# isarandi/metrabs

Measured on AMD Instinct MI355X. Metric: crops/sec (256px, 72 depth bins) at 1/2/4/8 MI355X; MPJPE vs ref, higher is better.
Workload: dtype f32

## Files before the change

include/metrabs_hip.h:

```cpp
#ifndef METRABS_HIP_H_
#define METRABS_HIP_H_

#include <stddef.h>
#include <stdint.h>

#ifdef __cplusplus
extern "C" {
#endif

#define MTR_VERSION 100

typedef void* mtr_stream_t;

enum mtr_dtype { MTR_F32 = 0, MTR_F16 = 1, MTR_BF16 = 2 };

enum mtr_layout {
  MTR_NCHW = 0,
  MTR_NHWC = 1
};

enum mtr_error {
  MTR_OK = 0,
  MTR_E_NULL = -1,
  MTR_E_SHAPE = -2,
// ... 172 lines not shown
                     const int32_t* row_start, const int32_t* sim_offsets, int n_images, int P, int A,
                     int J, const int32_t* edges, const float* mean_bones, int n_bones, int J_model,
                     const mtr_filter_params* params , void* workspace, size_t workspace_bytes,
                     int max_per_image, uint8_t* valid, int32_t* keep_idx, int32_t* keep_count,
                     mtr_stream_t stream);

int mtr_bias_act_nchw(void* y, int dtype, const float* bias , const void* residual, int act,
                      long long B, int C, int HW, mtr_stream_t stream);

int mtr_bias_act_rowmean_nchw(void* y, int dtype, const float* bias , int act, long long B,
                              int C, int HW, float* row_mean , mtr_stream_t stream);

int mtr_depthwise3x3_bias_act(const void* x, int dtype, const float* weight, const float* bias, int act,
                              long long B, int C, int H, int W, int stride, int pad, void* y,
                              float* row_mean, mtr_stream_t stream);
int mtr_depthwise3x3_bias_act_padded(const void* x, int dtype, const float* weight, const float* bias,
                                     int act, long long B, int C, int H, int W, int stride, int pad_top,
                                     int pad_left, int pad_bottom, int pad_right, void* y,
                                     float* row_mean, mtr_stream_t stream);

int mtr_depthwise5x5_bias_act_padded(const void* x, int dtype, const float* weight ,
                                     const float* bias, int act, long long B, int C, int H, int W,
                                     int stride, int pad_top, int pad_left, int pad_bottom, int pad_right,
                                     void* y, float* row_mean , mtr_stream_t stream);

int mtr_se_gate(const float* mean , const float* w1, const float* b1, const float* w2,
                const float* b2, int act, int gate_fn, int B, int C, int S, float* gate ,
                mtr_stream_t stream);

int mtr_conv1x1_bias_act(const void* x, int dtype, const float* weight, const float* bias,
                         const float* gate , const void* residual, int act, long long B,
                         int M, int K, int HW, void* y, mtr_stream_t stream);

int mtr_conv1x1_bias_act16(const void* x, int dtype, const void* weight, const float* bias,
                           const float* gate , const void* residual, int act, long long B,
                           int M, int K, int HW, void* y, mtr_stream_t stream);

int mtr_conv3x3_bias_act16(const void* x, int dtype, const void* weight , const float* bias,
                           const void* residual, int act, long long B, int Cin, int Cout, int H, int W, int stride,
                           void* y, mtr_stream_t stream);

size_t mtr_conv3x3_16_lds_bytes(long long B, int Cin, int Cout, int H, int W, int stride);

#ifdef __cplusplus
}
#endif
#endif
```

metrabs_amd/_lib.py:

```python
import ctypes
import os
from ctypes import POINTER, c_char_p, c_double, c_float, c_int, c_int32, c_size_t, c_uint8, c_void_p

LIB_PATH = os.path.join(os.path.dirname(os.path.abspath(__file__)), 'csrc', 'libmetrabs_hip.so')

MTR_F32, MTR_F16, MTR_BF16 = 0, 1, 2
MTR_NCHW, MTR_NHWC = 0, 1
MTR_WARP_PARAM_FLOATS = 36


class HeadParams(ctypes.Structure):
    _fields_ = [('proc_side', c_int32), ('stride_test', c_int32), ('centered_stride', c_int32),
                ('legacy_centered_stride_bug', c_int32), ('box_size_mm', c_float)]


class HeadOptions(ctypes.Structure):
    _fields_ = [('struct_size', ctypes.c_uint32),
                ('rt_tiles_per_workgroup', c_int32), ('groups_per_workgroup', c_int32),
                ('dma_staging', c_int32), ('rt_column_blocks', c_int32), ('rt_k_groups', c_int32),
                ('rt_loader', c_int32), ('rt_split_column_blocks', c_int32)]


def head_options(rt_tiles=0, groups_per_workgroup=0, dma_staging=-1, rt_column_blocks=0, rt_k_groups=0,
                 rt_loader=0, rt_split=0):
# ... 84 lines not shown
                                  c_void_p, c_void_p, c_void_p]),
    'mtr_postprocess_poses': (c_int, [c_void_p, c_void_p, c_void_p, c_void_p, c_void_p, c_int, c_void_p,
                                      c_int, c_void_p, c_void_p, c_void_p, c_int, c_int, c_int, c_int,
                                      c_void_p, c_void_p, c_void_p]),
    'mtr_linear_combine_points': (c_int, [c_void_p, c_void_p, c_int, c_int, c_int, c_void_p, c_void_p]),
    'mtr_warp_crops': (c_int, [c_void_p, c_void_p, c_void_p, c_int, c_int, c_int, c_void_p, c_int,
                               c_int, c_int, c_int, c_int, c_void_p, c_void_p]),
    'mtr_detector_geometry': (c_int, [c_int, c_int, c_int, POINTER(DetectorGeom)]),
    'mtr_detector_preprocess': (c_int, [c_void_p, c_int, c_int, c_int, POINTER(DetectorGeom), c_void_p,
                                        c_void_p]),
    'mtr_detector_preprocess_kernel': (c_int, [c_void_p, c_int, c_int, c_int, POINTER(DetectorGeom), c_int,
                                               c_void_p, c_void_p]),
    'mtr_detector_scale_boxes': (c_int, [c_void_p, c_int, POINTER(DetectorGeom), c_void_p, c_void_p]),
    'mtr_filter_poses_workspace_bytes': (ctypes.c_size_t, [c_int, c_int, c_int]),
    'mtr_filter_poses': (c_int, [c_void_p, c_void_p, c_void_p, c_void_p, c_void_p, c_int, c_int, c_int,
                                 c_int, c_void_p, c_void_p, c_int, c_int, POINTER(FilterParams), c_void_p,
                                 ctypes.c_size_t, c_int, c_void_p, c_void_p, c_void_p, c_void_p]),
    'mtr_depthwise3x3_bias_act': (c_int, [c_void_p, c_int, c_void_p, c_void_p, c_int, ctypes.c_longlong,
                                          c_int, c_int, c_int, c_int, c_int, c_void_p, c_void_p, c_void_p]),
    'mtr_depthwise3x3_bias_act_padded': (c_int, [c_void_p, c_int, c_void_p, c_void_p, c_int, ctypes.c_longlong,
                                                 c_int, c_int, c_int, c_int, c_int, c_int, c_int, c_int,
                                                 c_void_p, c_void_p, c_void_p]),
    'mtr_depthwise5x5_bias_act_padded': (c_int, [c_void_p, c_int, c_void_p, c_void_p, c_int, ctypes.c_longlong,
                                                 c_int, c_int, c_int, c_int, c_int, c_int, c_int, c_int,
                                                 c_void_p, c_void_p, c_void_p]),
    'mtr_bias_act_rowmean_nchw': (c_int, [c_void_p, c_int, c_void_p, c_int, ctypes.c_longlong, c_int, c_int,
                                          c_void_p, c_void_p]),
    'mtr_bias_act_nchw': (c_int, [c_void_p, c_int, c_void_p, c_void_p, c_int, ctypes.c_longlong, c_int,
                                  c_int, c_void_p]),
    'mtr_se_gate': (c_int, [c_void_p, c_void_p, c_void_p, c_void_p, c_void_p, c_int, c_int, c_int, c_int,
                            c_int, c_void_p, c_void_p]),
    'mtr_conv1x1_bias_act': (c_int, [c_void_p, c_int, c_void_p, c_void_p, c_void_p, c_void_p, c_int,
                                     ctypes.c_longlong, c_int, c_int, c_int, c_void_p, c_void_p]),
    'mtr_conv1x1_bias_act16': (c_int, [c_void_p, c_int, c_void_p, c_void_p, c_void_p, c_void_p, c_int,
                                       ctypes.c_longlong, c_int, c_int, c_int, c_void_p, c_void_p]),
    'mtr_conv3x3_bias_act16': (c_int, [c_void_p, c_int, c_void_p, c_void_p, c_void_p, c_int, ctypes.c_longlong,
                                       c_int, c_int, c_int, c_int, c_int, c_void_p, c_void_p]),
    'mtr_conv3x3_16_lds_bytes': (ctypes.c_size_t, [ctypes.c_longlong, c_int, c_int, c_int, c_int, c_int]),
}

_lib = None


def load(path=None):
    global _lib
    if _lib is not None and path is None:
        return _lib
    path = path or LIB_PATH
    import torch
    if not os.path.exists(path):
        raise RuntimeError(
            f'{path} not found: the HIP extension is not built. Run `python -m metrabs_amd.build` '
            f'(needs hipcc). metrabs_amd has no CPU fallback.')
    lib = ctypes.CDLL(path)
    for name, (restype, argtypes) in SIGNATURES.items():
        fn = getattr(lib, name)
        fn.restype = restype
        fn.argtypes = argtypes
    _lib = lib
    return lib


def check(code, what):
    if code != 0:
        msg = load().mtr_strerror(code).decode()
        raise RuntimeError(f'{what} failed: {msg} (code {code})')
# ... 22 lines not shown
```

metrabs_amd/backbones.py:

```python
import collections
import threading

import torch
import torch.nn.functional as F
from torch import nn


class DepthwiseConv2d(nn.Conv2d):

    use_miopen = False
    _backend_lock = threading.Lock()

    def forward(self, x):
        if x.is_cuda and not DepthwiseConv2d.use_miopen and torch.backends.cudnn.enabled:
            cudnn = torch.backends.cudnn
            with DepthwiseConv2d._backend_lock, cudnn.flags(
                    enabled=False, benchmark=cudnn.benchmark, deterministic=cudnn.deterministic,
                    allow_tf32=cudnn.allow_tf32):
                return super().forward(x)
        return super().forward(x)


class ConvBNAct(nn.Sequential):

# ... 49 lines not shown
            return False
        return (type(self.act) in (nn.SiLU, nn.ReLU) and type(self.gate) in self._GATE_NAMES
                and self.fc1.weight.dtype == torch.float32 and self.fc1.bias is not None
                and self.fc2.bias is not None and self.fc1.weight.is_cuda
                and self.fc1.in_channels % 4 == 0)


def _padded_conv(layers, name, cin, cout, k, stride, groups=1, act=nn.SiLU, bottomright=False):
    total = k - 1
    beg, end = total // 2, total - total // 2
    if bottomright:
        layers['padding'] = nn.ZeroPad2d((beg - 1, end + 1, beg - 1, end + 1))
        layers[name] = ConvBNAct(cin, cout, k, stride, groups=groups, act=act, padding=0)
    elif beg == end:
        layers[name] = ConvBNAct(cin, cout, k, stride, groups=groups, act=act, padding=beg)
    else:
        layers['padding'] = nn.ZeroPad2d((beg, end, beg, end))
        layers[name] = ConvBNAct(cin, cout, k, stride, groups=groups, act=act, padding=0)


class FusedMBConv(nn.Module):

    def __init__(self, cin, cout, expand, stride, bottomright=False):
        super().__init__()
        self.residual = stride == 1 and cin == cout
        mid = cin * expand
        layers = collections.OrderedDict()
        if expand == 1:
            _padded_conv(layers, '0', cin, cout, 3, stride, bottomright=bottomright)
        else:
            _padded_conv(layers, '0', cin, mid, 3, stride, bottomright=bottomright)
            layers['1'] = ConvBNAct(mid, cout, 1, 1, act=None)
        self.block = nn.Sequential(layers)

    def forward(self, x):
        return _block_plus_skip(self.block, x) if self.residual else self.block(x)


class MBConv(nn.Module):

    def __init__(self, cin, cout, expand, stride, k=3, bottomright=False):
        super().__init__()
        self.residual = stride == 1 and cin == cout
        mid = cin * expand
        layers = collections.OrderedDict()
        if mid != cin:
            layers['0'] = ConvBNAct(cin, mid, 1, 1)
        n = len(layers)
        _padded_conv(layers, str(n), mid, mid, k, stride, groups=mid, bottomright=bottomright)
        layers[str(n + 1)] = SqueezeExcite(mid, max(1, cin // 4))
        layers[str(n + 2)] = ConvBNAct(mid, cout, 1, 1, act=None)
        self.block = nn.Sequential(layers)

    def forward(self, x):
        return _block_plus_skip(self.block, x) if self.residual else self.block(x)


class Preproc(nn.Module):

    def forward(self, x):
        return x * 2 - 1


EFFNETV2 = {
    's': dict(stem=24, stages=[('f', 1, 1, 24, 24, 2), ('f', 4, 2, 24, 48, 4), ('f', 4, 2, 48, 64, 4),
                               ('m', 4, 2, 64, 128, 6), ('m', 6, 1, 128, 160, 9),
                               ('m', 6, 2, 160, 256, 15)], head=1280),
    'm': dict(stem=24, stages=[('f', 1, 1, 24, 24, 3), ('f', 4, 2, 24, 48, 5), ('f', 4, 2, 48, 80, 5),
                               ('m', 4, 2, 80, 160, 7), ('m', 6, 1, 160, 176, 14),
# ... 74 lines not shown
    layers += [ConvBNAct(cin, 960, 1, 1, act=nn.Hardswish), ConvBNAct(960, 1280, 1, 1, act=nn.Hardswish)]
    net = nn.Sequential(*layers)
    net.out_channels = 1280
    return net


def build_backbone(name):
    name = name.lower()
    if name in ('efficientnetv2-s', 'effnetv2-s', 'effv2s'):
        return efficientnetv2('s')
    if name in ('efficientnetv2-l', 'effnetv2-l', 'effv2l'):
        return efficientnetv2('l')
    if name in ('resnet18', 'resnet-18'):
        return resnet18()
    if name in ('mobilenetv3', 'mobilenetv3-large', 'mobilenet-v3'):
        return mobilenet_v3_large()
    raise ValueError(f'unknown backbone {name}')


_ACT_NAMES = {nn.SiLU: 'silu', nn.ReLU: 'relu', nn.Hardswish: 'hardswish'}


class ConvBiasAct(nn.Module):

    def __init__(self, conv, bias, act):
        super().__init__()
        self.conv = conv
        self.register_buffer('bias', bias.detach().float().contiguous())
        self.act = act
        self.act_name = None if act is None else _ACT_NAMES[type(act)]
        self.emit_mean = False
        self._mean = None
        self._gate = None
        self.last_path = None

    use_k13 = True
    k13_slower = frozenset({(960, 256, 64), (1536, 256, 64), (256, 1280, 64)})

    def k13_takes(self, x):
        c = self.conv
        if not (ConvBiasAct.use_k13 and not self.emit_mean and x.is_cuda and c.kernel_size == (1, 1)
                and c.stride == (1, 1) and c.padding == (0, 0) and c.dilation == (1, 1) and c.groups == 1
                and c.bias is None and c.padding_mode == 'zeros'):
            return False
        if torch.is_autocast_enabled('cuda') or (torch.is_grad_enabled() and c.weight.requires_grad):
            return False
        if x.dim() != 4 or (c.in_channels, c.out_channels, x.shape[2] * x.shape[3]) in ConvBiasAct.k13_slower:
            return False
        from . import kernels
        return kernels.conv1x1_supported(x, c.weight)

    use_k13h = True
    k13h_slower = frozenset({(192, 48, 4096), (256, 64, 1024), (1536, 256, 64), (256, 64, 9216), (768, 192, 576),
                             (1152, 224, 576), (1344, 224, 576), (1344, 384, 144), (2304, 384, 144),
                             (2304, 640, 144), (640, 3840, 144), (3840, 640, 144), (640, 1280, 144)})

    def k13h_takes(self, x):
        c = self.conv
        if not (ConvBiasAct.use_k13h and not self.emit_mean and x.is_cuda and x.dtype == c.weight.dtype
                and x.dtype in (torch.float16, torch.bfloat16) and c.kernel_size == (1, 1)
                and c.stride == (1, 1) and c.padding == (0, 0) and c.dilation == (1, 1) and c.groups == 1
                and c.bias is None and c.padding_mode == 'zeros'):
            return False
        if torch.is_autocast_enabled('cuda') or (torch.is_grad_enabled() and c.weight.requires_grad):
            return False
        if x.dim() != 4 or (c.in_channels, c.out_channels, x.shape[2] * x.shape[3]) in ConvBiasAct.k13h_slower:
            return False
        from . import kernels
        return kernels.conv1x1_16_supported(x, c.weight)

    def give_gate(self, x, gate):
        self._gate = (x, gate)

    def take_mean_f32(self, x):
        held, self._mean = self._mean, None
        if held is not None and held[0] is x:
            return held[1]
        return None

    def take_mean(self, x):
        m = self.take_mean_f32(x)
        return None if m is None else m.to(x.dtype).view(x.shape[0], x.shape[1], 1, 1)

    def forward(self, x, residual=None):
        held, self._gate = self._gate, None
        gate = held[1] if held is not None and held[0] is x else None
        w16 = self.conv.weight.dtype
        if x.dtype != w16 and w16 in (torch.float16, torch.bfloat16) and not torch.is_autocast_enabled(x.device.type):
            x = x.to(w16)
        if self.k13h_takes(x) and (residual is None or (residual.dtype == x.dtype and residual.is_contiguous()
                                                        and residual.data_ptr() % 16 == 0)):
            from . import kernels
            self.last_path = 'k13h' if gate is None else 'k13h_gate'
            return kernels.conv1x1_bias_act16(x, self.conv.weight, self.bias, self.act_name, gate=gate,
                                              residual=residual)
        if self.k13_takes(x) and (residual is None or (residual.dtype == x.dtype and residual.is_contiguous()
                                                       and residual.data_ptr() % 16 == 0)):
            from . import kernels
            self.last_path = 'k13' if gate is None else 'k13_gate'
            return kernels.conv1x1_bias_act(x, self.conv.weight, self.bias, self.act_name, gate=gate,
                                            residual=residual)
        self.last_path = 'library'
        if gate is not None:
            x = x * gate.to(x.dtype).view(x.shape[0], x.shape[1], 1, 1)
        return _library_conv_bias_act(self, x, residual)


def _library_conv_bias_act(mod, x, residual):
    y = mod.conv(x)
    hw_vec_ok = (y.shape[2] * y.shape[3]) % (16 // y.element_size()) == 0
    if y.is_cuda and y.is_contiguous() and hw_vec_ok and y.data_ptr() % 16 == 0 and (
            residual is None or (residual.dtype == y.dtype and residual.is_contiguous()
                                 and residual.data_ptr() % 16 == 0)):
        from . import kernels
        if getattr(mod, 'emit_mean', False) and residual is None:
            y, mean = kernels.bias_act_rowmean_(y, mod.bias, mod.act_name)
            mod._mean = (y, mean)
            return y
        return kernels.bias_act_(y, mod.bias, mod.act_name, residual)
    y = y + mod.bias.view(1, -1, 1, 1).to(y.dtype)
    y = y if mod.act is None else mod.act(y)
    return y if residual is None else residual + y


class Conv3x3BiasAct(nn.Module):

    use_k14h = True
    k14h_slower = frozenset({(64, 256, 2, 96, 96), (64, 64, 1, 64, 64)})

    def __init__(self, conv, bias, act):
        super().__init__()
        self.conv = conv
        from . import kernels
        self.register_buffer('weight_packed', kernels.pack_conv3x3_weight(conv.weight))
        self.register_buffer('bias', bias.detach().float().contiguous())
        self.act = act
        self.act_name = None if act is None else _ACT_NAMES[type(act)]
        self.stride = conv.stride[0]
        self.last_path = None

    @staticmethod
    def applies_to(conv):
# ... 187 lines not shown
```

metrabs_amd/csrc/conv1x1.hip:

```cpp
#include "common.h"

namespace mtr {

typedef float f32x16 __attribute__((ext_vector_type(16)));

constexpr int kC1PadX = 32;
constexpr int kC1PadW = 4;

template <int WM, int WN, int FM, int FN, int BK, int ACT>
__global__ __launch_bounds__(64 * WM * WN) void conv1x1_kernel(
    const float* __restrict__ x, const float* __restrict__ w, const float* __restrict__ bias,
    const float* __restrict__ gate, const float* __restrict__ residual, float* __restrict__ y, int M,
    int K, int HW, int n_total, FastDiv by_hw) {
  constexpr int NT = 64 * WM * WN;
  constexpr int BM = 32 * FM * WM, BN = 32 * FN * WN;
  constexpr int LDX = BN + kC1PadX, LDW = BM + kC1PadW;
  constexpr int XROW4 = BN / 4;
  constexpr int XPASS = NT / XROW4;
  constexpr int XV = (BK + XPASS - 1) / XPASS;
  constexpr int WPASS = NT / (BK / 4);
  constexpr int WV = (BM + WPASS - 1) / WPASS;
  static_assert(NT % XROW4 == 0 && NT % (BK / 4) == 0, "loader mapping");
  __shared__ float xs[2][BK * LDX];
  __shared__ float ws[2][BK * LDW];

  const int tid = threadIdx.x, lane = tid & 63, wave = tid >> 6;
  const int wm = wave % WM, wn = wave / WM;
  const int m0 = blockIdx.y * BM, n0 = blockIdx.x * BN;
  const long long khw = (long long)K * HW;

  const int xn4 = tid % XROW4, xk0 = tid / XROW4;
  const int xcol = n0 + xn4 * 4;
  const bool xcol_ok = xcol < n_total;
  const unsigned xb = xcol_ok ? fastdiv((unsigned)xcol, by_hw) : 0u;
  const float* xsrc = x + (long long)xb * khw + (xcol - (int)xb * HW);
  const float* gsrc = gate ? gate + (long long)xb * K : nullptr;
  const int wk4 = tid % (BK / 4), wr0 = tid / (BK / 4);

  float4 xr[XV], wr[WV];
  auto load_tile = [&](int k0) {
#pragma unroll
    for (int v = 0; v < XV; ++v) {
      const int k = k0 + xk0 + v * XPASS;
      float4 t = make_float4(0.0f, 0.0f, 0.0f, 0.0f);
      if (xcol_ok && k < K && xk0 + v * XPASS < BK) {
        t = *reinterpret_cast<const float4*>(xsrc + (long long)k * HW);
        if (gsrc) {
          const float g = gsrc[k];
          t.x *= g; t.y *= g; t.z *= g; t.w *= g;
        }
      }
      xr[v] = t;
    }
#pragma unroll
    for (int v = 0; v < WV; ++v) {
      const int m = m0 + wr0 + v * WPASS, k = k0 + wk4 * 4;
      float4 t = make_float4(0.0f, 0.0f, 0.0f, 0.0f);
      if (m < M && k < K && wr0 + v * WPASS < BM) t = *reinterpret_cast<const float4*>(w + (long long)m * K + k);
      wr[v] = t;
    }
  };
  auto store_tile = [&](int buf) {
#pragma unroll
    for (int v = 0; v < XV; ++v) {
      const int r = xk0 + v * XPASS;
      if (r < BK) *reinterpret_cast<float4*>(&xs[buf][r * LDX + xn4 * 4]) = xr[v];
    }
#pragma unroll
    for (int v = 0; v < WV; ++v) {
      const int r = wr0 + v * WPASS;
      if (r < BM) {
        float* d = &ws[buf][(wk4 * 4) * LDW + r];
        d[0] = wr[v].x; d[LDW] = wr[v].y; d[2 * LDW] = wr[v].z; d[3 * LDW] = wr[v].w;
      }
    }
  };

  f32x16 acc[FM][FN];
#pragma unroll
  for (int i = 0; i < FM; ++i)
#pragma unroll
    for (int j = 0; j < FN; ++j)
#pragma unroll
      for (int r = 0; r < 16; ++r) acc[i][j][r] = 0.0f;

  const int half = lane >> 5, l32 = lane & 31;
  const int n_tiles = (K + BK - 1) / BK;
  load_tile(0);
  store_tile(0);
  __syncthreads();
  for (int t = 0; t < n_tiles; ++t) {
    const int buf = t & 1;
    if (t + 1 < n_tiles) load_tile((t + 1) * BK);
    const float* xb_ = &xs[buf][half * LDX + wn * (32 * FN) + l32];
    const float* wb_ = &ws[buf][half * LDW + wm * (32 * FM) + l32];
#pragma unroll
    for (int kk = 0; kk < BK; kk += 2) {
      float a[FN], b[FM];
#pragma unroll
      for (int j = 0; j < FN; ++j) a[j] = xb_[kk * LDX + j * 32];
#pragma unroll
      for (int i = 0; i < FM; ++i) b[i] = wb_[kk * LDW + i * 32];
#pragma unroll
      for (int i = 0; i < FM; ++i)
#pragma unroll
        for (int j = 0; j < FN; ++j) acc[i][j] = __builtin_amdgcn_mfma_f32_32x32x2f32(a[j], b[i], acc[i][j], 0, 0, 0);
    }
    if (t + 1 < n_tiles) store_tile(buf ^ 1);
    __syncthreads();
  }

#pragma unroll
  for (int i = 0; i < FM; ++i) {
    const int m = m0 + wm * (32 * FM) + i * 32 + l32;
    if (m >= M) continue;
    const float bm = bias[m];
#pragma unroll
    for (int j = 0; j < FN; ++j) {
#pragma unroll
      for (int g = 0; g < 4; ++g) {
        const int col = n0 + wn * (32 * FN) + j * 32 + 8 * g + 4 * half;
        if (col >= n_total) continue;
        const unsigned b = fastdiv((unsigned)col, by_hw);
        const long long off = ((long long)b * M + m) * HW + (col - (int)b * HW);
        float4 r;
        r.x = activate<ACT>(acc[i][j][4 * g + 0] + bm);
        r.y = activate<ACT>(acc[i][j][4 * g + 1] + bm);
        r.z = activate<ACT>(acc[i][j][4 * g + 2] + bm);
        r.w = activate<ACT>(acc[i][j][4 * g + 3] + bm);
        if (residual) {
          const float4 q = *reinterpret_cast<const float4*>(residual + off);
          r.x += q.x; r.y += q.y; r.z += q.z; r.w += q.w;
        }
        *reinterpret_cast<float4*>(y + off) = r;
      }
    }
  }
}

enum Conv1x1Config { kCfgWide = 0, kCfgSquare = 1, kCfgTall = 2 };

struct Conv1x1Plan { int cfg, waves_m, bm, bn; };

inline Conv1x1Plan pick_config(int M, int K, int HW, long long B) {
  const long long n_total = B * HW;
  const long long n_tiles128 = (n_total + 127) / 128;
  if (M <= 160) {
    const int w = (M + 31) / 32;
    return {kCfgTall, w, 32 * w, 32};
  }
  if (M == 256 && K >= 512) return {kCfgTall, 4, 128, 32};
  if (M % 192 == 0 && (M / 192) * n_tiles128 >= 512) return {kCfgWide, 2, 192, 128};
  return {kCfgSquare, 2, 128, 128};
}

template <int WM, int WN, int FM, int FN, int BK>
static int launch_conv1x1_cfg(const float* x, const float* w, const float* bias, const float* gate,
                              const float* residual, float* y, int act, int M, int K, int HW,
                              long long n_total, hipStream_t stream) {
  constexpr int BM = 32 * FM * WM, BN = 32 * FN * WN;
  const long long gx = (n_total + BN - 1) / BN, gy = (M + BM - 1) / BM;
  if (gx > 0x7fffffffLL || gy > 65535) return MTR_E_SHAPE;
  const dim3 grid((unsigned)gx, (unsigned)gy), block(64 * WM * WN);
  const FastDiv by_hw = make_fastdiv((unsigned)HW);
  MTR_CLEAR_STALE();
#define MTR_C1_LAUNCH(ACT)                                                                                    \
  hipLaunchKernelGGL((conv1x1_kernel<WM, WN, FM, FN, BK, ACT>), grid, block, 0, stream, x, w, bias, gate, residual, \
                     y, M, K, HW, (int)n_total, by_hw)
  switch (act) {
    case kActNone: MTR_C1_LAUNCH(kActNone); break;
    case kActRelu: MTR_C1_LAUNCH(kActRelu); break;
    case kActSilu: MTR_C1_LAUNCH(kActSilu); break;
    case kActHardswish: MTR_C1_LAUNCH(kActHardswish); break;
    default: return MTR_E_PARAM;
  }
#undef MTR_C1_LAUNCH
  MTR_CHECK_LAUNCH();
  return MTR_OK;
}

}

extern "C" int mtr_conv1x1_bias_act(const void* x, int dtype, const float* weight, const float* bias,
                                    const float* gate, const void* residual, int act, long long B, int M,
                                    int K, int HW, void* y, mtr_stream_t stream) {
  if (!x || !weight || !bias || !y) return MTR_E_NULL;
  if (dtype != MTR_F32) return MTR_E_DTYPE;
  if (B < 0 || M <= 0 || K <= 0 || HW <= 0) return MTR_E_SHAPE;
  if (HW % 4 || K % 4) return MTR_E_SHAPE;
  if (B * HW > 0x7fffffffLL || (long long)K * HW > 0x7fffffffLL || (long long)M * HW > 0x7fffffffLL)
    return MTR_E_SHAPE;
  if (act < mtr::kActNone || act > mtr::kActHardswish) return MTR_E_PARAM;
  if (((uintptr_t)x % 16) || ((uintptr_t)weight % 16) || ((uintptr_t)y % 16) || ((uintptr_t)residual % 16))
    return MTR_E_ALIGN;
  if (x == y || (residual && residual == x)) return MTR_E_PARAM;
  if (B == 0) return MTR_OK;
  const float* xf = (const float*)x;
  const float* rf = (const float*)residual;
  float* yf = (float*)y;
  const long long n_total = B * HW;
  hipStream_t s = (hipStream_t)stream;
  const mtr::Conv1x1Plan p = mtr::pick_config(M, K, HW, B);
  switch (p.cfg) {
    case mtr::kCfgWide:
      return mtr::launch_conv1x1_cfg<2, 2, 3, 2, 16>(xf, weight, bias, gate, rf, yf, act, M, K, HW, n_total, s);
    case mtr::kCfgSquare:
      return mtr::launch_conv1x1_cfg<2, 2, 2, 2, 16>(xf, weight, bias, gate, rf, yf, act, M, K, HW, n_total, s);
    default:
      switch (p.waves_m) {
        case 1: return mtr::launch_conv1x1_cfg<1, 1, 1, 1, 16>(xf, weight, bias, gate, rf, yf, act, M, K, HW, n_total, s);
        case 2: return mtr::launch_conv1x1_cfg<2, 1, 1, 1, 16>(xf, weight, bias, gate, rf, yf, act, M, K, HW, n_total, s);
        case 3: return mtr::launch_conv1x1_cfg<3, 1, 1, 1, 16>(xf, weight, bias, gate, rf, yf, act, M, K, HW, n_total, s);
        case 4: return mtr::launch_conv1x1_cfg<4, 1, 1, 1, 32>(xf, weight, bias, gate, rf, yf, act, M, K, HW, n_total, s);
        default: return mtr::launch_conv1x1_cfg<5, 1, 1, 1, 16>(xf, weight, bias, gate, rf, yf, act, M, K, HW, n_total, s);
      }
  }
}
```

metrabs_amd/kernels.py:

```python
import ctypes

import torch

from metrabs_amd import _lib
from metrabs_amd._lib import check, current_stream_ptr, dtype_code, require_cuda


def _ptr(t):
    return ctypes.c_void_p(t.data_ptr()) if t is not None else ctypes.c_void_p(0)


def softargmax_decode(logits, n_points, cfg, out=None, nhwc_staging=0):
    require_cuda(logits)
    lib = _lib.load()
    nhwc = _is_channels_last(logits)
    if not nhwc:
        logits = logits.contiguous()
    B, n_out, H, W = logits.shape
    J = int(n_points)
    D = n_out // J - 1
    if n_out != J * (1 + D) or D != cfg.depth:
        raise ValueError(f'logits have {n_out} channels, expected J*(1+depth) = {J * (1 + cfg.depth)}')
    if out is None:
        c2d = torch.empty(B, J, 2, device=logits.device, dtype=torch.float32)
# ... 504 lines not shown
        current_stream_ptr(x.device)), 'mtr_depthwise5x5_bias_act_padded')
    return (y, mean) if want_mean else y



SE_GATE_CODES = {'sigmoid': 0, 'hardsigmoid': 1}


def se_gate(mean, w1, b1, w2, b2, act, gate_fn, out=None):
    require_cuda(mean, w1, b1, w2, b2)
    B, C = mean.shape[0], mean.shape[1]
    S = w1.shape[0]
    w1, w2 = w1.reshape(S, -1), w2.reshape(C, -1)
    if mean.dtype != torch.float32 or mean.numel() != B * C or w1.shape[1] != C or w2.shape[1] != S:
        raise ValueError('se_gate: mean [B, C] f32, w1 [S, C], w2 [C, S]')
    tensors = [t.contiguous().float() for t in (mean, w1, b1, w2, b2)]
    if out is None:
        out = torch.empty(B, C, device=mean.device, dtype=torch.float32)
    check(_lib.load().mtr_se_gate(*(_ptr(t) for t in tensors), ACT_CODES[act], SE_GATE_CODES[gate_fn], B, C, S,
                                  _ptr(out), current_stream_ptr(mean.device)), 'mtr_se_gate')
    return out



def conv1x1_supported(x, weight):
    if x.dim() != 4 or x.dtype != torch.float32 or weight.dtype != torch.float32 or not x.is_contiguous():
        return False
    K, HW = x.shape[1], x.shape[2] * x.shape[3]
    return (weight.numel() == weight.shape[0] * K and HW % 4 == 0 and K % 4 == 0
            and x.data_ptr() % 16 == 0 and weight.data_ptr() % 16 == 0
            and x.shape[0] * HW < 2 ** 31 and K * HW < 2 ** 31 and weight.shape[0] * HW < 2 ** 31)


def conv1x1_bias_act(x, w, bias, act, gate=None, residual=None, out=None):
    require_cuda(x, w, bias, gate, residual)
    B, K, H, W = x.shape
    M = w.shape[0]
    w = w.reshape(M, -1)
    if w.shape[1] != K:
        raise ValueError(f'conv1x1_bias_act: weight has {w.shape[1]} input channels, x has {K}')
    if gate is not None and (gate.dtype != torch.float32 or gate.numel() != B * K):
        raise ValueError('conv1x1_bias_act: gate must be [B, Cin] f32')
    if residual is not None and (residual.shape != (B, M, H, W) or residual.dtype != x.dtype
                                 or not residual.is_contiguous()):
        raise ValueError('conv1x1_bias_act: residual must be [B, Cout, H, W] like the output, contiguous')
    if out is None:
        out = torch.empty(B, M, H, W, device=x.device, dtype=x.dtype)
    elif out.shape != (B, M, H, W) or out.dtype != x.dtype or not out.is_contiguous():
        raise ValueError('conv1x1_bias_act: out must be [B, Cout, H, W] like the output, contiguous')
    check(_lib.load().mtr_conv1x1_bias_act(
        _ptr(x), dtype_code(x.dtype), _ptr(w.contiguous()), _ptr(bias.contiguous().float()),
        None if gate is None else _ptr(gate.contiguous()), None if residual is None else _ptr(residual),
        ACT_CODES[act], B, M, K, H * W, _ptr(out), current_stream_ptr(x.device)), 'mtr_conv1x1_bias_act')
    return out



def conv1x1_16_supported(x, weight):
    if x.dim() != 4 or x.dtype not in (torch.float16, torch.bfloat16) or weight.dtype != x.dtype \
            or not x.is_contiguous() or not weight.is_contiguous():
        return False
    K, HW = x.shape[1], x.shape[2] * x.shape[3]
    return (weight.numel() == weight.shape[0] * K and HW % 8 == 0 and K % 8 == 0
            and x.data_ptr() % 16 == 0 and weight.data_ptr() % 16 == 0
            and x.shape[0] * HW < 2 ** 31 and K * HW < 2 ** 31 and weight.shape[0] * HW < 2 ** 31)


def conv1x1_bias_act16(x, w, bias, act, gate=None, residual=None, out=None):
    require_cuda(x, w, bias, gate, residual)
    B, K, H, W = x.shape
    M = w.shape[0]
    w = w.reshape(M, -1)
    if w.shape[1] != K:
        raise ValueError(f'conv1x1_bias_act16: weight has {w.shape[1]} input channels, x has {K}')
    if w.dtype != x.dtype:
        raise ValueError(f'conv1x1_bias_act16: weight is {w.dtype}, x is {x.dtype}')
    if gate is not None and (gate.dtype != torch.float32 or gate.numel() != B * K):
        raise ValueError('conv1x1_bias_act16: gate must be [B, Cin] f32')
    if residual is not None and (residual.shape != (B, M, H, W) or residual.dtype != x.dtype
                                 or not residual.is_contiguous()):
        raise ValueError('conv1x1_bias_act16: residual must be [B, Cout, H, W] like the output, contiguous')
    if out is None:
# ... 56 lines not shown
```

Before: 8112.

## Defer FusedMBConv bias+activation into the projection conv1x1 prologue and pipeline tiles

After: 8591 (median of 6 runs). 5.9% higher.

```diff
diff --git a/include/metrabs_hip.h b/include/metrabs_hip.h
--- a/include/metrabs_hip.h
+++ b/include/metrabs_hip.h
@@ -228,6 +228,13 @@
                          const float* gate , const void* residual, int act, long long B,
                          int M, int K, int HW, void* y, mtr_stream_t stream);
 
+int mtr_conv1x1_bias_act_pre(const void* x, int dtype, const float* weight, const float* bias,
+                             const float* gate , const void* residual, int act,
+                             const float* in_bias , int in_act, long long B, int M, int K, int HW,
+                             void* y, mtr_stream_t stream);
+
+int mtr_conv1x1_plan(long long B, int M, int K, int HW, int* plan );
+
 int mtr_conv1x1_bias_act16(const void* x, int dtype, const void* weight, const float* bias,
                            const float* gate , const void* residual, int act, long long B,
                            int M, int K, int HW, void* y, mtr_stream_t stream);
diff --git a/metrabs_amd/_lib.py b/metrabs_amd/_lib.py
--- a/metrabs_amd/_lib.py
+++ b/metrabs_amd/_lib.py
@@ -140,6 +140,9 @@
                             c_int, c_void_p, c_void_p]),
     'mtr_conv1x1_bias_act': (c_int, [c_void_p, c_int, c_void_p, c_void_p, c_void_p, c_void_p, c_int,
                                      ctypes.c_longlong, c_int, c_int, c_int, c_void_p, c_void_p]),
+    'mtr_conv1x1_bias_act_pre': (c_int, [c_void_p, c_int, c_void_p, c_void_p, c_void_p, c_void_p, c_int, c_void_p,
+                                         c_int, ctypes.c_longlong, c_int, c_int, c_int, c_void_p, c_void_p]),
+    'mtr_conv1x1_plan': (c_int, [ctypes.c_longlong, c_int, c_int, c_int, c_void_p]),
     'mtr_conv1x1_bias_act16': (c_int, [c_void_p, c_int, c_void_p, c_void_p, c_void_p, c_void_p, c_int,
                                        ctypes.c_longlong, c_int, c_int, c_int, c_void_p, c_void_p]),
     'mtr_conv3x3_bias_act16': (c_int, [c_void_p, c_int, c_void_p, c_void_p, c_void_p, c_int, ctypes.c_longlong,
diff --git a/metrabs_amd/backbones.py b/metrabs_amd/backbones.py
--- a/metrabs_amd/backbones.py
+++ b/metrabs_amd/backbones.py
@@ -105,9 +105,32 @@
             _padded_conv(layers, '0', cin, mid, 3, stride, bottomright=bottomright)
             layers['1'] = ConvBNAct(mid, cout, 1, 1, act=None)
         self.block = nn.Sequential(layers)
-
-    def forward(self, x):
-        return _block_plus_skip(self.block, x) if self.residual else self.block(x)
+        self.last_deferred = False
+
+    defer_epilogue = True
+
+    def _deferral_pair(self):
+        kids = list(self.block)
+        if len(kids) < 2 or not all(isinstance(k, ConvBNAct) for k in kids[-2:]):
+            return None
+        (c3, *rest3), (pj, *restp) = kids[-2], kids[-1]
+        if type(c3) is not ConvBiasAct or type(pj) is not ConvBiasAct or c3.emit_mean or \
+                not all(isinstance(m, nn.Identity) for m in rest3 + restp):
+            return None
+        return c3, pj
+
+    def forward(self, x):
+        pair = self._deferral_pair() if FusedMBConv.defer_epilogue else None
+        if pair is None:
+            self.last_deferred = False
+            return _block_plus_skip(self.block, x) if self.residual else self.block(x)
+        c3, pj = pair
+        y = x
+        for m in list(self.block)[:-2]:
+            y = m(y)
+        y = c3(y, defer_to=pj)
+        self.last_deferred = pj.holds_pre(y)
+        return pj(y, residual=x if self.residual else None)
 
 
 class MBConv(nn.Module):
@@ -248,10 +271,14 @@
         self.emit_mean = False
         self._mean = None
         self._gate = None
+        self._pre = None
         self.last_path = None
+        self.last_pre = False
 
     use_k13 = True
-    k13_slower = frozenset({(960, 256, 64), (1536, 256, 64), (256, 1280, 64)})
+    k13_slower = frozenset({(960, 256, 64), (1536, 256, 64), (256, 1280, 64),
+                            (384, 96, 2304), (384, 192, 576), (768, 192, 576), (1152, 224, 576), (1344, 224, 576),
+                            (1344, 384, 144), (2304, 384, 144), (3840, 640, 144), (640, 1280, 144)})
 
     def k13_takes(self, x):
         c = self.conv
@@ -288,6 +315,12 @@
     def give_gate(self, x, gate):
         self._gate = (x, gate)
 
+    def give_pre(self, x, bias, act_name):
+        self._pre = (x, bias, act_name)
+
+    def holds_pre(self, x):
+        return self._pre is not None and self._pre[0] is x
+
     def take_mean_f32(self, x):
         held, self._mean = self._mean, None
         if held is not None and held[0] is x:
@@ -298,32 +331,55 @@
         m = self.take_mean_f32(x)
         return None if m is None else m.to(x.dtype).view(x.shape[0], x.shape[1], 1, 1)
 
-    def forward(self, x, residual=None):
+    def forward(self, x, residual=None, defer_to=None):
         held, self._gate = self._gate, None
         gate = held[1] if held is not None and held[0] is x else None
+        held, self._pre = self._pre, None
+        pre = held[1:] if held is not None and held[0] is x else None
+        res_ok = residual is None or (residual.dtype == x.dtype and residual.is_contiguous()
+                                      and residual.data_ptr() % 16 == 0)
+        if pre is not None and not (gate is None and res_ok and self.k13_takes(x)):
+            x, pre = _bias_act(x, pre[0], pre[1]), None
+        self.last_pre = pre is not None
         w16 = self.conv.weight.dtype
         if x.dtype != w16 and w16 in (torch.float16, torch.bfloat16) and not torch.is_autocast_enabled(x.device.type):
             x = x.to(w16)
-        if self.k13h_takes(x) and (residual is None or (residual.dtype == x.dtype and residual.is_contiguous()
-                                                        and residual.data_ptr() % 16 == 0)):
+        if res_ok and self.k13h_takes(x):
             from . import kernels
             self.last_path = 'k13h' if gate is None else 'k13h_gate'
             return kernels.conv1x1_bias_act16(x, self.conv.weight, self.bias, self.act_name, gate=gate,
                                               residual=residual)
-        if self.k13_takes(x) and (residual is None or (residual.dtype == x.dtype and residual.is_contiguous()
-                                                       and residual.data_ptr() % 16 == 0)):
+        if res_ok and (pre is not None or self.k13_takes(x)):
             from . import kernels
             self.last_path = 'k13' if gate is None else 'k13_gate'
             return kernels.conv1x1_bias_act(x, self.conv.weight, self.bias, self.act_name, gate=gate,
-                                            residual=residual)
+                                            residual=residual, pre=pre)
         self.last_path = 'library'
         if gate is not None:
             x = x * gate.to(x.dtype).view(x.shape[0], x.shape[1], 1, 1)
+        if defer_to is not None and residual is None and not self.emit_mean:
+            y = self.conv(x)
+            if defer_to.k13_takes(y) and not y.requires_grad:
+                defer_to.give_pre(y, self.bias, self.act_name)
+                return y
+            return _library_epilogue(self, y, None)
         return _library_conv_bias_act(self, x, residual)
 
 
+def _bias_act(y, bias, act_name):
+    hw_vec_ok = (y.shape[2] * y.shape[3]) % (16 // y.element_size()) == 0
+    if y.is_cuda and y.is_contiguous() and hw_vec_ok and y.data_ptr() % 16 == 0 and not y.requires_grad:
+        from . import kernels
+        return kernels.bias_act_(y, bias, act_name, None)
+    y = y + bias.view(1, -1, 1, 1).to(y.dtype)
+    return y if act_name is None else {'silu': F.silu, 'relu': F.relu, 'hardswish': F.hardswish}[act_name](y)
+
+
 def _library_conv_bias_act(mod, x, residual):
-    y = mod.conv(x)
+    return _library_epilogue(mod, mod.conv(x), residual)
+
+
+def _library_epilogue(mod, y, residual):
     hw_vec_ok = (y.shape[2] * y.shape[3]) % (16 // y.element_size()) == 0
     if y.is_cuda and y.is_contiguous() and hw_vec_ok and y.data_ptr() % 16 == 0 and (
             residual is None or (residual.dtype == y.dtype and residual.is_contiguous()
diff --git a/metrabs_amd/csrc/conv1x1.hip b/metrabs_amd/csrc/conv1x1.hip
--- a/metrabs_amd/csrc/conv1x1.hip
+++ b/metrabs_amd/csrc/conv1x1.hip
@@ -7,11 +7,13 @@
 constexpr int kC1PadX = 32;
 constexpr int kC1PadW = 4;
 
-template <int WM, int WN, int FM, int FN, int BK, int ACT>
+enum Conv1x1In { kInPlain = 0, kInGate = 1, kInPre = 2 };
+
+template <int WM, int WN, int FM, int FN, int BK, int ACT, int IN>
 __global__ __launch_bounds__(64 * WM * WN) void conv1x1_kernel(
     const float* __restrict__ x, const float* __restrict__ w, const float* __restrict__ bias,
-    const float* __restrict__ gate, const float* __restrict__ residual, float* __restrict__ y, int M,
-    int K, int HW, int n_total, FastDiv by_hw) {
+    const float* __restrict__ in_vec, const float* __restrict__ residual, float* __restrict__ y, int M, int K,
+    int HW, int n_total, FastDiv by_hw) {
   constexpr int NT = 64 * WM * WN;
   constexpr int BM = 32 * FM * WM, BN = 32 * FN * WN;
   constexpr int LDX = BN + kC1PadX, LDW = BM + kC1PadW;
@@ -20,8 +22,9 @@
   constexpr int XV = (BK + XPASS - 1) / XPASS;
   constexpr int WPASS = NT / (BK / 4);
   constexpr int WV = (BM + WPASS - 1) / WPASS;
-  static_assert(NT % XROW4 == 0 && NT % (BK / 4) == 0, "loader mapping");
-  __shared__ float xs[2][BK * LDX];
+  static_assert(NT % XROW4 == 0 && NT % (BK / 4) == 0 && BM % WPASS == 0, "loader mapping");
+  constexpr bool XSPARE = XV * XPASS != BK;
+  __shared__ float xs[2][(BK + (XSPARE ? 1 : 0)) * LDX];
   __shared__ float ws[2][BK * LDW];
 
   const int tid = threadIdx.x, lane = tid & 63, wave = tid >> 6;
@@ -33,48 +36,54 @@
   const int xcol = n0 + xn4 * 4;
   const bool xcol_ok = xcol < n_total;
   const unsigned xb = xcol_ok ? fastdiv((unsigned)xcol, by_hw) : 0u;
-  const float* xsrc = x + (long long)xb * khw + (xcol - (int)xb * HW);
-  const float* gsrc = gate ? gate + (long long)xb * K : nullptr;
+  const float* xsrc = x + (xcol_ok ? (long long)xb * khw + (xcol - (int)xb * HW) : 0LL);
+  const float* vsrc = IN == kInGate ? in_vec + (long long)xb * K : in_vec;
   const int wk4 = tid % (BK / 4), wr0 = tid / (BK / 4);
 
-  float4 xr[XV], wr[WV];
-  auto load_tile = [&](int k0) {
+  struct Regs { float4 x[XV]; float v[XV]; float4 w[WV]; };
+  auto load_tile = [&](int k0, Regs& r) {
 #pragma unroll
     for (int v = 0; v < XV; ++v) {
-      const int k = k0 + xk0 + v * XPASS;
-      float4 t = make_float4(0.0f, 0.0f, 0.0f, 0.0f);
-      if (xcol_ok && k < K && xk0 + v * XPASS < BK) {
-        t = *reinterpret_cast<const float4*>(xsrc + (long long)k * HW);
-        if (gsrc) {
-          const float g = gsrc[k];
+      const int k = min(k0 + xk0 + v * XPASS, K - 1);
+      r.x[v] = *reinterpret_cast<const float4*>(xsrc + (long long)k * HW);
+      if constexpr (IN != kInPlain) r.v[v] = vsrc[k];
+    }
+#pragma unroll
+    for (int v = 0; v < WV; ++v) {
+      const int m = min(m0 + wr0 + v * WPASS, M - 1), k = min(k0 + wk4 * 4, K - 4);
+      r.w[v] = *reinterpret_cast<const float4*>(w + (long long)m * K + k);
+    }
+  };
+  auto store_tile = [&](int buf, int k0, const Regs& r) {
+#pragma unroll
+    for (int v = 0; v < XV; ++v) {
+      const int row = xk0 + v * XPASS;
+      {
+        float4 t = r.x[v];
+        if constexpr (IN == kInGate) {
+          const float g = r.v[v];
           t.x *= g; t.y *= g; t.z *= g; t.w *= g;
         }
+        if constexpr (IN >= kInPre) {
+          const float b = r.v[v];
+          t.x = activate<IN - kInPre>(t.x + b); t.y = activate<IN - kInPre>(t.y + b);
+          t.z = activate<IN - kInPre>(t.z + b); t.w = activate<IN - kInPre>(t.w + b);
+        }
+        if (!(xcol_ok && k0 + row < K)) t = make_float4(0.0f, 0.0f, 0.0f, 0.0f);
+        *reinterpret_cast<float4*>(&xs[buf][(XSPARE ? min(row, BK) : row) * LDX + xn4 * 4]) = t;
       }
-      xr[v] = t;
     }
 #pragma unroll
     for (int v = 0; v < WV; ++v) {
-      const int m = m0 + wr0 + v * WPASS, k = k0 + wk4 * 4;
-      float4 t = make_float4(0.0f, 0.0f, 0.0f, 0.0f);
-      if (m < M && k < K && wr0 + v * WPASS < BM) t = *reinterpret_cast<const float4*>(w + (long long)m * K + k);
-      wr[v] = t;
+      const int row = wr0 + v * WPASS;
+      {
+        float4 t = r.w[v];
+        if (!(m0 + row < M && k0 + wk4 * 4 < K)) t = make_float4(0.0f, 0.0f, 0.0f, 0.0f);
+        float* d = &ws[buf][(wk4 * 4) * LDW + row];
+        d[0] = t.x; d[LDW] = t.y; d[2 * LDW] = t.z; d[3 * LDW] = t.w;
+      }
     }
   };
-  auto store_tile = [&](int buf) {
-#pragma unroll
-    for (int v = 0; v < XV; ++v) {
-      const int r = xk0 + v * XPASS;
-      if (r < BK) *reinterpret_cast<float4*>(&xs[buf][r * LDX + xn4 * 4]) = xr[v];
-    }
-#pragma unroll
-    for (int v = 0; v < WV; ++v) {
-      const int r = wr0 + v * WPASS;
-      if (r < BM) {
-        float* d = &ws[buf][(wk4 * 4) * LDW + r];
-        d[0] = wr[v].x; d[LDW] = wr[v].y; d[2 * LDW] = wr[v].z; d[3 * LDW] = wr[v].w;
-      }
-    }
-  };
 
   f32x16 acc[FM][FN];
 #pragma unroll
@@ -85,13 +94,7 @@
       for (int r = 0; r < 16; ++r) acc[i][j][r] = 0.0f;
 
   const int half = lane >> 5, l32 = lane & 31;
-  const int n_tiles = (K + BK - 1) / BK;
-  load_tile(0);
-  store_tile(0);
-  __syncthreads();
-  for (int t = 0; t < n_tiles; ++t) {
-    const int buf = t & 1;
-    if (t + 1 < n_tiles) load_tile((t + 1) * BK);
+  auto multiply = [&](int buf) {
     const float* xb_ = &xs[buf][half * LDX + wn * (32 * FN) + l32];
     const float* wb_ = &ws[buf][half * LDW + wm * (32 * FM) + l32];
 #pragma unroll
@@ -106,9 +109,43 @@
 #pragma unroll
         for (int j = 0; j < FN; ++j) acc[i][j] = __builtin_amdgcn_mfma_f32_32x32x2f32(a[j], b[i], acc[i][j], 0, 0, 0);
     }
-    if (t + 1 < n_tiles) store_tile(buf ^ 1);
+  };
+
+  const int n_tiles = (K + BK - 1) / BK;
+  Regs ra, rb;
+  load_tile(0, ra);
+  if (n_tiles > 1) load_tile(BK, rb);
+  store_tile(0, 0, ra);
+  __syncthreads();
+  int t = 0;
+  for (; t + 4 <= n_tiles; t += 2) {
+    load_tile((t + 2) * BK, ra);
+    __builtin_amdgcn_sched_barrier(0);
+    multiply(0);
+    __builtin_amdgcn_sched_barrier(0);
+    store_tile(1, (t + 1) * BK, rb);
     __syncthreads();
-  }
+    load_tile((t + 3) * BK, rb);
+    __builtin_amdgcn_sched_barrier(0);
+    multiply(1);
+    __builtin_amdgcn_sched_barrier(0);
+    store_tile(0, (t + 2) * BK, ra);
+    __syncthreads();
+  }
+  if (t + 2 <= n_tiles) {
+    const bool third = t + 2 < n_tiles;
+    if (third) load_tile((t + 2) * BK, ra);
+    multiply(0);
+    store_tile(1, (t + 1) * BK, rb);
+    __syncthreads();
+    multiply(1);
+    if (third) {
+      store_tile(0, (t + 2) * BK, ra);
+      __syncthreads();
+    }
+    t += 2;
+  }
+  if (t < n_tiles) multiply(0);
 
 #pragma unroll
   for (int i = 0; i < FM; ++i) {
@@ -138,36 +175,55 @@
   }
 }
 
-enum Conv1x1Config { kCfgWide = 0, kCfgSquare = 1, kCfgTall = 2 };
-
-struct Conv1x1Plan { int cfg, waves_m, bm, bn; };
+enum Conv1x1Config { kCfgWide = 0, kCfgSquare = 1, kCfgTall = 2, kCfgFlat = 3 };
+
+struct Conv1x1Plan { int cfg, waves_m, bm, bn, bk; };
 
 inline Conv1x1Plan pick_config(int M, int K, int HW, long long B) {
   const long long n_total = B * HW;
   const long long n_tiles128 = (n_total + 127) / 128;
+  if (M <= 64 && HW >= 1024) {
+    const int w = (M + 31) / 32;
+    return {kCfgFlat, w, 32 * w, 128, 16};
+  }
   if (M <= 160) {
     const int w = (M + 31) / 32;
-    return {kCfgTall, w, 32 * w, 32};
-  }
-  if (M == 256 && K >= 512) return {kCfgTall, 4, 128, 32};
-  if (M % 192 == 0 && (M / 192) * n_tiles128 >= 512) return {kCfgWide, 2, 192, 128};
-  return {kCfgSquare, 2, 128, 128};
-}
+    return {kCfgTall, w, 32 * w, 32, w == 4 ? 32 : 16};
+  }
+  if (M == 256 && K >= 512) return {kCfgTall, 4, 128, 32, 32};
+  if (M % 192 == 0 && (M / 192) * n_tiles128 >= 512) return {kCfgWide, 2, 192, 128, 16};
+  return {kCfgSquare, 2, 128, 128, 16};
+}
+
+struct Conv1x1Args {
+  const float *x, *w, *bias, *in_vec, *residual;
+  float* y;
+  int in_mode, act, M, K, HW;
+  long long n_total;
+  hipStream_t stream;
+};
 
 template <int WM, int WN, int FM, int FN, int BK>
-static int launch_conv1x1_cfg(const float* x, const float* w, const float* bias, const float* gate,
-                              const float* residual, float* y, int act, int M, int K, int HW,
-                              long long n_total, hipStream_t stream) {
+static int launch_conv1x1_cfg(const Conv1x1Args& a) {
   constexpr int BM = 32 * FM * WM, BN = 32 * FN * WN;
-  const long long gx = (n_total + BN - 1) / BN, gy = (M + BM - 1) / BM;
+  const long long gx = (a.n_total + BN - 1) / BN, gy = (a.M + BM - 1) / BM;
   if (gx > 0x7fffffffLL || gy > 65535) return MTR_E_SHAPE;
   const dim3 grid((unsigned)gx, (unsigned)gy), block(64 * WM * WN);
-  const FastDiv by_hw = make_fastdiv((unsigned)HW);
+  const FastDiv by_hw = make_fastdiv((unsigned)a.HW);
   MTR_CLEAR_STALE();
-#define MTR_C1_LAUNCH(ACT)                                                                                    \
-  hipLaunchKernelGGL((conv1x1_kernel<WM, WN, FM, FN, BK, ACT>), grid, block, 0, stream, x, w, bias, gate, residual, \
-                     y, M, K, HW, (int)n_total, by_hw)
-  switch (act) {
+#define MTR_C1_LAUNCH_IN(ACT, IN)                                                                                  \
+  hipLaunchKernelGGL((conv1x1_kernel<WM, WN, FM, FN, BK, ACT, IN>), grid, block, 0, a.stream, a.x, a.w, a.bias,     \
+                     a.in_vec, a.residual, a.y, a.M, a.K, a.HW, (int)a.n_total, by_hw)
+#define MTR_C1_LAUNCH(ACT)                                       \
+  switch (a.in_mode) {                                           \
+    case kInGate: MTR_C1_LAUNCH_IN(ACT, kInGate); break;         \
+    case kInPre + kActNone: MTR_C1_LAUNCH_IN(ACT, kInPre + kActNone); break;           \
+    case kInPre + kActRelu: MTR_C1_LAUNCH_IN(ACT, kInPre + kActRelu); break;           \
+    case kInPre + kActSilu: MTR_C1_LAUNCH_IN(ACT, kInPre + kActSilu); break;           \
+    case kInPre + kActHardswish: MTR_C1_LAUNCH_IN(ACT, kInPre + kActHardswish); break; \
+    default: MTR_C1_LAUNCH_IN(ACT, kInPlain); break;             \
+  }
+  switch (a.act) {
     case kActNone: MTR_C1_LAUNCH(kActNone); break;
     case kActRelu: MTR_C1_LAUNCH(kActRelu); break;
     case kActSilu: MTR_C1_LAUNCH(kActSilu); break;
@@ -175,44 +231,75 @@
     default: return MTR_E_PARAM;
   }
 #undef MTR_C1_LAUNCH
+#undef MTR_C1_LAUNCH_IN
   MTR_CHECK_LAUNCH();
   return MTR_OK;
 }
 
-}
-
-extern "C" int mtr_conv1x1_bias_act(const void* x, int dtype, const float* weight, const float* bias,
-                                    const float* gate, const void* residual, int act, long long B, int M,
-                                    int K, int HW, void* y, mtr_stream_t stream) {
+static int check_conv1x1(const void* x, int dtype, const float* weight, const float* bias, const void* residual,
+                         int act, long long B, int M, int K, int HW, const void* y) {
   if (!x || !weight || !bias || !y) return MTR_E_NULL;
   if (dtype != MTR_F32) return MTR_E_DTYPE;
   if (B < 0 || M <= 0 || K <= 0 || HW <= 0) return MTR_E_SHAPE;
   if (HW % 4 || K % 4) return MTR_E_SHAPE;
   if (B * HW > 0x7fffffffLL || (long long)K * HW > 0x7fffffffLL || (long long)M * HW > 0x7fffffffLL)
     return MTR_E_SHAPE;
-  if (act < mtr::kActNone || act > mtr::kActHardswish) return MTR_E_PARAM;
+  if (act < kActNone || act > kActHardswish) return MTR_E_PARAM;
   if (((uintptr_t)x % 16) || ((uintptr_t)weight % 16) || ((uintptr_t)y % 16) || ((uintptr_t)residual % 16))
     return MTR_E_ALIGN;
   if (x == y || (residual && residual == x)) return MTR_E_PARAM;
-  if (B == 0) return MTR_OK;
-  const float* xf = (const float*)x;
-  const float* rf = (const float*)residual;
-  float* yf = (float*)y;
-  const long long n_total = B * HW;
-  hipStream_t s = (hipStream_t)stream;
-  const mtr::Conv1x1Plan p = mtr::pick_config(M, K, HW, B);
+  return MTR_OK;
+}
+
+static int dispatch_conv1x1(const Conv1x1Args& a, long long B) {
+  const Conv1x1Plan p = pick_config(a.M, a.K, a.HW, B);
   switch (p.cfg) {
-    case mtr::kCfgWide:
-      return mtr::launch_conv1x1_cfg<2, 2, 3, 2, 16>(xf, weight, bias, gate, rf, yf, act, M, K, HW, n_total, s);
-    case mtr::kCfgSquare:
-      return mtr::launch_conv1x1_cfg<2, 2, 2, 2, 16>(xf, weight, bias, gate, rf, yf, act, M, K, HW, n_total, s);
+    case kCfgWide: return launch_conv1x1_cfg<2, 2, 3, 2, 16>(a);
+    case kCfgSquare: return launch_conv1x1_cfg<2, 2, 2, 2, 16>(a);
+    case kCfgFlat: return p.waves_m == 1 ? launch_conv1x1_cfg<1, 2, 1, 2, 16>(a) : launch_conv1x1_cfg<2, 2, 1, 2, 16>(a);
     default:
       switch (p.waves_m) {
-        case 1: return mtr::launch_conv1x1_cfg<1, 1, 1, 1, 16>(xf, weight, bias, gate, rf, yf, act, M, K, HW, n_total, s);
-        case 2: return mtr::launch_conv1x1_cfg<2, 1, 1, 1, 16>(xf, weight, bias, gate, rf, yf, act, M, K, HW, n_total, s);
-        case 3: return mtr::launch_conv1x1_cfg<3, 1, 1, 1, 16>(xf, weight, bias, gate, rf, yf, act, M, K, HW, n_total, s);
-        case 4: return mtr::launch_conv1x1_cfg<4, 1, 1, 1, 32>(xf, weight, bias, gate, rf, yf, act, M, K, HW, n_total, s);
-        default: return mtr::launch_conv1x1_cfg<5, 1, 1, 1, 16>(xf, weight, bias, gate, rf, yf, act, M, K, HW, n_total, s);
+        case 1: return launch_conv1x1_cfg<1, 1, 1, 1, 16>(a);
+        case 2: return launch_conv1x1_cfg<2, 1, 1, 1, 16>(a);
+        case 3: return launch_conv1x1_cfg<3, 1, 1, 1, 16>(a);
+        case 4: return launch_conv1x1_cfg<4, 1, 1, 1, 32>(a);
+        default: return launch_conv1x1_cfg<5, 1, 1, 1, 16>(a);
       }
   }
 }
+
+}
+
+extern "C" int mtr_conv1x1_bias_act(const void* x, int dtype, const float* weight, const float* bias,
+                                    const float* gate, const void* residual, int act, long long B, int M,
+                                    int K, int HW, void* y, mtr_stream_t stream) {
+  const int rc = mtr::check_conv1x1(x, dtype, weight, bias, residual, act, B, M, K, HW, y);
+  if (rc != MTR_OK || B == 0) return rc;
+  const mtr::Conv1x1Args a{(const float*)x, weight, bias, gate, (const float*)residual, (float*)y,
+                           gate ? mtr::kInGate : mtr::kInPlain, act, M, K, HW, B * HW,
+                           (hipStream_t)stream};
+  return mtr::dispatch_conv1x1(a, B);
+}
+
+extern "C" int mtr_conv1x1_bias_act_pre(const void* x, int dtype, const float* weight, const float* bias,
+                                        const float* gate, const void* residual, int act,
+                                        const float* in_bias, int in_act, long long B, int M, int K, int HW,
+                                        void* y, mtr_stream_t stream) {
+  if (!in_bias) return MTR_E_NULL;
+  const int rc = mtr::check_conv1x1(x, dtype, weight, bias, residual, act, B, M, K, HW, y);
+  if (rc != MTR_OK) return rc;
+  if (in_act < mtr::kActNone || in_act > mtr::kActHardswish) return MTR_E_PARAM;
+  if (gate) return MTR_E_PARAM;
+  if (B == 0) return MTR_OK;
+  const mtr::Conv1x1Args a{(const float*)x, weight, bias, in_bias, (const float*)residual, (float*)y,
+                           mtr::kInPre + in_act, act, M, K, HW, B * HW, (hipStream_t)stream};
+  return mtr::dispatch_conv1x1(a, B);
+}
+
+extern "C" int mtr_conv1x1_plan(long long B, int M, int K, int HW, int* plan) {
+  if (!plan) return MTR_E_NULL;
+  if (B < 0 || M <= 0 || K <= 0 || HW <= 0) return MTR_E_SHAPE;
+  const mtr::Conv1x1Plan p = mtr::pick_config(M, K, HW, B);
+  plan[0] = p.cfg; plan[1] = p.waves_m; plan[2] = p.bm; plan[3] = p.bn; plan[4] = p.bk;
+  return MTR_OK;
+}
diff --git a/metrabs_amd/kernels.py b/metrabs_amd/kernels.py
--- a/metrabs_amd/kernels.py
+++ b/metrabs_amd/kernels.py
@@ -560,7 +560,14 @@
             and x.shape[0] * HW < 2 ** 31 and K * HW < 2 ** 31 and weight.shape[0] * HW < 2 ** 31)
 
 
-def conv1x1_bias_act(x, w, bias, act, gate=None, residual=None, out=None):
+def conv1x1_plan(B, M, K, HW):
+    plan = (ctypes.c_int * 5)()
+    check(_lib.load().mtr_conv1x1_plan(B, M, K, HW, plan), 'mtr_conv1x1_plan')
+    return dict(config=('wide', 'square', 'tall', 'flat')[plan[0]], waves_m=plan[1], bm=plan[2], bn=plan[3],
+                bk=plan[4])
+
+
+def conv1x1_bias_act(x, w, bias, act, gate=None, residual=None, out=None, pre=None):
     require_cuda(x, w, bias, gate, residual)
     B, K, H, W = x.shape
     M = w.shape[0]
@@ -576,6 +583,17 @@
         out = torch.empty(B, M, H, W, device=x.device, dtype=x.dtype)
     elif out.shape != (B, M, H, W) or out.dtype != x.dtype or not out.is_contiguous():
         raise ValueError('conv1x1_bias_act: out must be [B, Cout, H, W] like the output, contiguous')
+    if pre is not None:
+        in_bias, in_act = pre
+        require_cuda(in_bias)
+        if in_bias.dtype != torch.float32 or in_bias.numel() != K or not in_bias.is_contiguous():
+            raise ValueError('conv1x1_bias_act: pre must be (in_bias [Cin] f32 contiguous, in_act)')
+        check(_lib.load().mtr_conv1x1_bias_act_pre(
+            _ptr(x), dtype_code(x.dtype), _ptr(w.contiguous()), _ptr(bias.contiguous().float()),
+            None if gate is None else _ptr(gate.contiguous()), None if residual is None else _ptr(residual),
+            ACT_CODES[act], _ptr(in_bias), ACT_CODES[in_act], B, M, K, H * W, _ptr(out),
+            current_stream_ptr(x.device)), 'mtr_conv1x1_bias_act_pre')
+        return out
     check(_lib.load().mtr_conv1x1_bias_act(
         _ptr(x), dtype_code(x.dtype), _ptr(w.contiguous()), _ptr(bias.contiguous().float()),
         None if gate is None else _ptr(gate.contiguous()), None if residual is None else _ptr(residual),
```
